# open-mmlab/Amphion

Hardware: AMD Instinct MI355X
Metric: audio samples/sec (HiFi-GAN V1 22.05 kHz generator, mel->wav) (higher is better)
Workload: dtype f32 (split-f16 MFMA: 3 x v_mfma_f32_32x32x16_f16 per term, f32 accumulate)

## Files before the change

amphion_amd/_lib.py:

```python
from __future__ import annotations

import ctypes
import os
import weakref
from ctypes import POINTER, c_char_p, c_float, c_int, c_int32, c_int64, c_size_t, c_void_p

_HERE = os.path.dirname(os.path.abspath(__file__))
LIB_PATH = os.environ.get("AMP_LIB_PATH") or os.path.join(_HERE, "lib", "libamphion_hip.so")

AMP_MAX_STAGES = 8
AMP_MAX_KERNELS = 8
AMP_MAX_DILATIONS = 8

AMP_ARCH_HIFIGAN, AMP_ARCH_BIGVGAN, AMP_ARCH_HIFIGAN_VITS = 0, 1, 2
AMP_ACT_LRELU, AMP_ACT_SNAKE, AMP_ACT_SNAKEBETA = 0, 1, 2
AMP_PRECISION_F32, AMP_PRECISION_F16X3 = 0, 1
AMP_CONV_OPT_PAD_REFLECT, AMP_CONV_OPT_TANH = 1, 2
AMP_PAD_REPLICATE, AMP_PAD_ZEROS, AMP_PAD_REFLECT = 0, 1, 2
AMP_PW_BIAS, AMP_PW_BIAS_GELU, AMP_PW_SCALE_RES = 0, 1, 2
PRECISIONS = {"f32": AMP_PRECISION_F32, "fp32": AMP_PRECISION_F32, "f16x3": AMP_PRECISION_F16X3}


class AmpError(RuntimeError):

# ... 219 lines not shown
    "amp_embed_tokens": (c_int, [c_void_p, c_void_p, c_void_p, c_int, c_int, c_int, c_int, c_float, c_void_p, c_void_p]),
    "amp_embed_sum_c": (c_int, [c_void_p, c_int, POINTER(c_void_p), POINTER(c_int), c_int, c_void_p, c_int, c_int, c_void_p, c_void_p, c_void_p]),
    "amp_embed_sum_check": (c_int, [c_void_p, c_void_p]),
    "amp_durations": (c_int, [c_void_p, c_void_p, c_int, c_int, c_float, c_void_p, c_void_p, c_void_p, c_void_p]),
    "amp_expand_path": (c_int, [c_void_p, c_void_p, c_void_p, c_void_p, c_int, c_int, c_int, c_int, c_void_p, c_void_p, c_void_p]),
    "amp_expand_path_strided": (c_int, [c_void_p, ctypes.c_longlong, c_void_p, c_void_p, c_void_p, c_int, c_int, c_int, c_int, c_void_p, c_void_p, c_void_p]),
    "amp_gauss_sample": (c_int, [c_void_p, c_void_p, c_void_p, c_size_t, c_float, c_void_p, c_void_p]),
    "amp_snake": (c_int, [c_void_p, c_int, c_int, c_int, c_void_p, c_void_p, c_int, c_void_p, c_void_p]),
    "amp_fir_upsample": (c_int, [c_void_p, c_int, c_int, c_int, c_void_p, c_int, c_int, c_void_p, c_void_p]),
    "amp_fir_filter": (c_int, [c_void_p, c_int, c_int, c_int, c_void_p, c_int, c_int, c_int, c_int, c_int, c_void_p, c_void_p]),
    "amp_wav_to_pcm16": (c_int, [c_void_p, c_int, c_int, ctypes.c_longlong, c_void_p, c_void_p, ctypes.c_longlong, c_void_p]),
    "amp_conv_set_option": (c_int, [c_void_p, c_int, c_int]),
    "amp_pair_forward": (c_int, [c_void_p, c_void_p, c_void_p, c_int, c_int, c_float, c_void_p, c_void_p]),
    "amp_resblock_forward": (c_int, [POINTER(c_void_p), POINTER(c_void_p), c_int, c_void_p, c_int, c_int, c_float, c_void_p, c_void_p]),
    "amp_set_resblock_fusion": (c_int, [c_int]),
    "amp_conv_destroy": (None, [c_void_p]),
    "amp_set_small_conv": (c_int, [c_int]),
    "amp_set_conv_blk": (c_int, [c_int]),
    "amp_set_conv_rg_fast": (c_int, [c_int]),
    "amp_set_pingpong": (c_int, [c_int]),
    "amp_set_conv_blk_narrow": (c_int, [c_int]),
    "amp_ampblock_forward": (c_int, [POINTER(c_void_p), POINTER(c_void_p), c_int, c_void_p, c_void_p, c_int, c_void_p, c_void_p,
                                     c_void_p, c_int, c_int, c_void_p, c_int, c_float, c_void_p]),
    "amp_set_ampblock_fusion": (c_int, [c_int]),
    "amp_conv_create_gated": (c_int, [c_int, c_int, c_int, c_int, c_void_p, c_void_p, POINTER(c_void_p)]),
    "amp_wn_forward": (c_int, [POINTER(c_void_p), POINTER(c_void_p), c_int, c_void_p, c_void_p, ctypes.c_longlong, c_void_p, c_int, c_int,
                               c_void_p, c_void_p, c_void_p]),
    "amp_wn_gate": (c_int, [c_void_p, c_void_p, ctypes.c_longlong, c_void_p, c_int, c_int, c_int, c_void_p]),
    "amp_wn_accumulate": (c_int, [c_void_p, c_void_p, c_void_p, c_void_p, c_int, c_int, c_int, c_int, c_int, c_void_p]),
    "amp_sequence_mask": (c_int, [c_void_p, c_void_p, c_int, c_int, c_int, c_void_p]),
# ... 136 lines not shown
```

amphion_amd/csrc/amp_host.h:

```cpp
#pragma once
#include <math.h>

#include <vector>

#include "amp_internal.h"

#define AMP_HIP(expr)                                                                  \
    do {                                                                               \
        hipError_t e__ = (expr);                                                       \
        if (e__ != hipSuccess) {                                                       \
            set_error("%s failed: %s (%s:%d)", #expr, hipGetErrorString(e__), __FILE__, __LINE__); \
            return AMP_ERR_HIP;                                                        \
        }                                                                              \
    } while (0)

#define AMP_RC(expr) do { int rc__ = (expr); if (rc__ != AMP_OK) return rc__; } while (0)

struct amp_conv {
    int transposed = 0, cin = 0, cout = 0, k = 0, stride = 1, dilation = 1, padding = 0;
    int M = 0, ntaps = 0, KT = 0, off0 = 0, dstep = 0, halo_left = 0, halo_right = 0, up = 1, up_pad = 0;
    int nchunks = 0;
    int precision = amp::PREC_F32;
    int pad_reflect = 0, tanh_out = 0;
    int out_pad = 0;
// ... 42 lines not shown
        return AMP_OK;
    }
    template <class T, class P>
    int upload(const std::vector<T>& v, P** out) { return upload(v.data(), v.size() * sizeof(T), (void**)out); }
};

int default_precision();

constexpr int kConvBlkDefault = 3;
constexpr int kConvRgFastDefault = 1;
constexpr int kPingPongDefault = 1;
struct Config {
    int pair_strips = -1;
    int strip_fit = -1;
    int rb_fusion = 1;
    int ampb_fusion = 1;
    int conv_blk = kConvBlkDefault;
    size_t group_bytes = 0;
    int small_conv = 1;
    int conv_rg_fast = 1;
    int pingpong = 1;
    int narrow_blk = 1;
    int rb_streams = -1;
    Config();
};
Config& cfg();

struct RangeGuard {
    unsigned* dev = nullptr;
    unsigned* host = nullptr;
// ... 53 lines not shown

int conv_build(amp_conv* c, const float* w, const float* bias);
int conv_run(const amp_conv* c, const float* x, int B, int T, float slope_in, const float* res, float slope_out, float* y, int mode, float div,
             hipStream_t stream, long long xbs = 0, const int* lens = nullptr, int len_mul = 1, ConvArgs* plan_small = nullptr,
             int* plan_ni = nullptr);
int next_rev(const int* lens);

bool pair_supported(const amp_conv* c1, const amp_conv* c2);
int pair_run(const amp_conv* c1, const amp_conv* c2, const float* x, int B, int T, float slope, float* y, int mode, float div,
             hipStream_t stream, const int* lens = nullptr, int len_mul = 1);
bool pair_strip_plan(int B, int T, int k, bool ragged, int* form, int* strip_len, int* spi, int* steps);
bool pair_tile_args(const amp_conv* c1, const amp_conv* c2, const float* x, int B, int T, float slope, float* y, int mode, float div,
                    const int* lens, int len_mul, PairArgs* out);

bool rb_supported(const amp_conv* const* c1, const amp_conv* const* c2, int np, int B, int T);
int rb_split(const amp_conv* const* c1, int np, int B, int T);
int rb_run(const amp_conv* const* c1, const amp_conv* const* c2, int np, const float* x, int B, int T, float slope, float* y, int mode,
           float div, hipStream_t stream, const int* lens = nullptr, int len_mul = 1, int first = 0, int count = -1);

struct ActParams {
    float* a_dev = nullptr;
    float* invb_dev = nullptr;
    float* fu_dev = nullptr;
    float* fd_dev = nullptr;
    float* fu2_dev = nullptr;
};
int act_params_upload(const float* alpha_dev, const float* beta_dev, int C, int logscale, const float* filt_up_host,
                      const float* filt_down_host, float** out);
bool ampb_supported(const amp_conv* const* c1, const amp_conv* const* c2, int np, const ActParams* acts, size_t nacts, int B, int T);
int ampb_run(const amp_conv* const* c1, const amp_conv* const* c2, int np, const ActParams* acts, const float* x, int B, int T, float* y,
             int mode, float div, hipStream_t stream, const int* lens = nullptr, int len_mul = 1);
// ... 3 lines not shown
```

amphion_amd/csrc/amp_internal.h:

```cpp
#pragma once
#include <hip/hip_runtime.h>
#include <stdarg.h>
#include <stdint.h>
#include <stdio.h>

#include <atomic>
#include <mutex>
#include <string>
#include <vector>

#include "amphion_hip.h"

namespace amp {

constexpr int KC = 8;
constexpr int KC16 = 16;

enum { PREC_F32 = 0, PREC_F16X3 = 1 };

struct ConvArgs {
    const float* x;
    const void* wp;
    const float* bias;
    const float* res;
// ... 65 lines not shown
};
hipError_t launch_pair3(const Pair3Args& p, hipStream_t stream);

constexpr int AMP_RB_MAX_PAIRS = 3;
struct RbArgs {
    const float* x;
    float* y;
    const void* wp1[AMP_RB_MAX_PAIRS];
    const float* bias1[AMP_RB_MAX_PAIRS];
    const void* wp2[AMP_RB_MAX_PAIRS];
    const float* bias2[AMP_RB_MAX_PAIRS];
    float sc1[AMP_RB_MAX_PAIRS], isc1[AMP_RB_MAX_PAIRS], sc2[AMP_RB_MAX_PAIRS], isc2[AMP_RB_MAX_PAIRS];
    int dil[AMP_RB_MAX_PAIRS];
    int np;
    int rh;
    int B, C, T;
    int tiles_per_item;
    int rev;
    float slope;
    int mode;
    float div;
    const int* lens;
    int len_mul;
    unsigned* range_flag;
};

constexpr int AMP_AMPB_MAX_STEPS = 6;
struct AmpbArgs {
    const float* x;
    float* y;
// ... 249 lines not shown
```

amphion_amd/csrc/conv_host.hip:

```cpp
#include <string.h>

#include <memory>
#include <type_traits>
#include <vector>

#include "amp_host.h"

namespace amp {

template <int... K> struct Taps { static constexpr int list[] = {K...}; };
using ConvTaps = Taps<1, 2, 3, 5, 7, 11>;
using BlkTaps = Taps<2, 3, 7, 11>;
using SmallTaps = Taps<1, 3, 5, 7, 11>;
using PairTaps = Taps<3, 5, 7, 11>;
using RbTaps = Taps<3, 5, 7, 11>;
using AmpbTaps = Taps<3, 5, 7, 11>;

template <int... K, typename R, typename F>
static R with_taps(Taps<K...>, int k, R dflt, F&& f) {
    R r = dflt;
    (void)((k == K && (r = f(std::integral_constant<int, K>{}), true)) || ...);
    return r;
}

// ... 380 lines not shown
    *out = a;
    return true;
}

static int rb_fusion_mode() { return cfg().rb_fusion; }
static int rb_form(int C, int k) {
    const int m = rb_fusion_mode();
    if (m == 0) return -1;
    if (m == 3) return (C == 32 || (C == 64 && k <= 5)) ? 0 : 1;
    if (m == 2) return 1;
    if (C == 32) return k >= 11 ? 1 : 0;
    if (C == 64) return k <= 5 ? 0 : 1;
    if (C == 128) return 1;
    return -1;
}
constexpr long long kRbMinWorkgroups = 256;

bool rb_supported(const amp_conv* const* c1, const amp_conv* const* c2, int np, int B, int T) {
    if (np < 1 || np > AMP_RB_MAX_PAIRS) return false;
    int max_dil = 1, rh = 0;
    for (int p = 0; p < np; ++p) {
        if (!c1[p] || !c2[p] || !pair_supported(c1[p], c2[p])) return false;
        if (c1[p]->cin != c1[0]->cin || c1[p]->k != c1[0]->k) return false;
        max_dil = c1[p]->dilation > max_dil ? c1[p]->dilation : max_dil;
        rh += (c1[p]->k - 1) / 2 * (c1[p]->dilation + 1);
    }
    const int form = rb_form(c1[0]->cin, c1[0]->k);
    if (form < 0) return false;
    const int W = rb_tile(c1[0]->k, c1[0]->cin, max_dil, form);
    if (W <= 0 || W - 2 * rh < W / 2) return false;
    const int NT = W - 2 * rh;
    if (rb_fusion_mode() == 1 && (long long)B * ((T + NT - 1) / NT) < kRbMinWorkgroups) return false;
    return true;
}

int rb_split(const amp_conv* const* c1, int np, int B, int T) {
    if (np != 3 || rb_fusion_mode() != 1) return 0;
    int max_dil = 1, rh = 0;
    for (int p = 0; p < np; ++p) {
        max_dil = c1[p]->dilation > max_dil ? c1[p]->dilation : max_dil;
        rh += (c1[p]->k - 1) / 2 * (c1[p]->dilation + 1);
    }
    const int W = rb_tile(c1[0]->k, c1[0]->cin, max_dil, rb_form(c1[0]->cin, c1[0]->k));
    const int NT = W - 2 * rh;
    if (W <= 0 || 5 * NT >= 4 * W) return 0;
    if ((long long)B * ((T + NT - 1) / NT) < 1024) return 0;
    return 2;
}

int rb_run(const amp_conv* const* c1, const amp_conv* const* c2, int np, const float* x, int B, int T, float slope, float* y, int mode,
           float div, hipStream_t stream, const int* lens, int len_mul, int first, int count) {
    if (x == y) { set_error("rb_run: x and y must not alias"); return AMP_ERR_INVALID; }
    if (slope > 1.f) { set_error("rb_run: leaky_relu slope %g > 1 is outside the fused kernels", (double)slope); return AMP_ERR_UNSUPPORTED; }
    RbArgs a{};
    a.x = x; a.y = y;
    a.np = count < 0 ? np - first : count;
    c1 += first;
    c2 += first;
    int max_dil = 1;
    for (int p = 0; p < a.np; ++p) {
        a.wp1[p] = c1[p]->wp_dev; a.bias1[p] = c1[p]->bias_dev; a.wp2[p] = c2[p]->wp_dev; a.bias2[p] = c2[p]->bias_dev;
        a.sc1[p] = 16.f * c1[p]->wscale; a.isc1[p] = 1.f / a.sc1[p];
        a.sc2[p] = 16.f * c2[p]->wscale; a.isc2[p] = 1.f / a.sc2[p];
        a.dil[p] = c1[p]->dilation;
        a.rh += (c1[p]->k - 1) / 2 * (c1[p]->dilation + 1);
        max_dil = c1[p]->dilation > max_dil ? c1[p]->dilation : max_dil;
    }
    for (int p = a.np; p < AMP_RB_MAX_PAIRS; ++p) {
        a.wp1[p] = a.wp1[0]; a.bias1[p] = a.bias1[0]; a.wp2[p] = a.wp2[0]; a.bias2[p] = a.bias2[0]; a.dil[p] = 1;
    }
    a.B = B; a.C = c1[0]->cin; a.T = T;
    const int form = rb_form(a.C, c1[0]->k);
    const int W = rb_tile(c1[0]->k, a.C, max_dil, form);
    const int NT = W - 2 * a.rh;
    a.tiles_per_item = (T + NT - 1) / NT;
    a.slope = slope; a.mode = mode; a.div = div;
    a.lens = lens; a.len_mul = len_mul;
    a.range_flag = range_flag_for_current_device();
    a.rev = next_rev(lens);
    AMP_HIP(launch_rb(c1[0]->k, a, form, stream));
    return AMP_OK;
}

static int ampb_fusion_mode() { return cfg().ampb_fusion; }
static int ampb_form(int C, int k) {
    const int m = ampb_fusion_mode();
    if (m == 0) return -1;
    if (m == 3) return C == 32 ? 0 : 1;
    if (m == 2) return 1;
    if (C == 32) return k >= 11 ? 1 : 0;
    if (C == 64) return k <= 3 ? 1 : -1;
    return -1;
}
constexpr long long kAmpbMinWorkgroups = 256;

// ... 220 lines not shown
}

int amp_resblock_forward(const amp_conv* const* c1, const amp_conv* const* c2, int n_pairs, const float* x_dev, int B, int T,
                         float slope, float* y_dev, void* stream) {
    if (!c1 || !c2 || !x_dev || !y_dev) { set_error("amp_resblock_forward: null argument"); return AMP_ERR_INVALID; }
    if (B <= 0 || T <= 0 || n_pairs < 1 || n_pairs > AMP_RB_MAX_PAIRS) { set_error("amp_resblock_forward: B=%d T=%d n_pairs=%d", B, T, n_pairs); return AMP_ERR_INVALID; }
    for (int p = 0; p < n_pairs; ++p) if (!c1[p] || !c2[p]) { set_error("amp_resblock_forward: null conv handle"); return AMP_ERR_INVALID; }
    if (!rb_supported(c1, c2, n_pairs, B, T)) {
        set_error("amp_resblock_forward: block (C=%d k=%d, %d pairs, B=%d T=%d) is not covered by the whole-resblock kernel under the "
                  "current amp_set_resblock_fusion mode", c1[0]->cin, c1[0]->k, n_pairs, B, T);
        return AMP_ERR_UNSUPPORTED;
    }
    return rb_run(c1, c2, n_pairs, x_dev, B, T, slope, y_dev, 0, 1.f, (hipStream_t)stream);
}

int amp_ampblock_forward(const amp_conv* const* c1, const amp_conv* const* c2, int n_pairs, const float* alpha_dev,
                         const float* beta_dev, int logscale, const float* filt_up_host, const float* filt_down_host,
                         const float* x_dev, int B, int T, float* y_dev, int mode, float div, void* stream) {
    if (!c1 || !c2 || !alpha_dev || !filt_up_host || !filt_down_host || !x_dev || !y_dev) { set_error("amp_ampblock_forward: null argument"); return AMP_ERR_INVALID; }
    if (B <= 0 || T <= 0 || n_pairs < 1 || 2 * n_pairs > AMP_AMPB_MAX_STEPS || mode < 0 || mode > 2) {
        set_error("amp_ampblock_forward: B=%d T=%d n_pairs=%d mode=%d", B, T, n_pairs, mode);
        return AMP_ERR_INVALID;
    }
    if (x_dev == y_dev) { set_error("amp_ampblock_forward: x and y must not alias (tiles read each other's halo)"); return AMP_ERR_INVALID; }
    for (int p = 0; p < n_pairs; ++p) if (!c1[p] || !c2[p]) { set_error("amp_ampblock_forward: null conv handle"); return AMP_ERR_INVALID; }
    const int C = c1[0]->cin, na = 2 * n_pairs;
    float* scratch[AMP_AMPB_MAX_STEPS] = {};
    ActParams acts[AMP_AMPB_MAX_STEPS];
    int rc = AMP_OK;
    for (int i = 0; i < na && rc == AMP_OK; ++i) {
// ... 42 lines not shown
```

amphion_amd/csrc/generator.hip:

```cpp
#include <math.h>
#include <stdio.h>

#include <map>
#include <memory>
#include <mutex>
#include <string>
#include <vector>

#include "amp_host.h"

using namespace amp;

struct HostTensor {
    std::vector<int64_t> shape;
    std::vector<float> data;
    size_t numel() const { size_t n = 1; for (auto s : shape) n *= (size_t)s; return n; }
};

struct ResBlock {
    int k = 0;
    std::vector<int> dil;
    std::vector<std::unique_ptr<amp_conv>> c1, c2;
    std::vector<ActParams> acts;
};
// ... 540 lines not shown
    *ran = true;
    return AMP_OK;
}

static int wait_before_last(hipEvent_t wait, hipStream_t sj) {
    if (wait) AMP_HIP(hipStreamWaitEvent(sj, wait, 0));
    return AMP_OK;
}

static int run_resblock1(const Stage& s, const ResBlock& rb, const RbBufs& b, int mode_last, hipEvent_t wait, hipStream_t sj) {
    const int B = s.B, t = s.t;
    const float nk = (float)s.g->d.n_kernels;
    const int nd = (int)rb.dil.size();
    RbPtrs q(rb);
    if (q.n && rb_supported(q.c1, q.c2, nd, B, t)) {
        const int sp = rb_split(q.c1, nd, B, t);
        if (sp > 0) AMP_RC(rb_run(q.c1, q.c2, nd, s.U, B, t, kLreluSlope, b.R, 0, 1.f, sj, s.lens, s.lm, 0, sp));
        AMP_RC(wait_before_last(wait, sj));
        return rb_run(q.c1, q.c2, nd, sp > 0 ? b.R : s.U, B, t, kLreluSlope, b.XS, mode_last, nk, sj, s.lens, s.lm, sp, -1);
    }
    const float* cur = s.U;
    for (int p = 0; p < nd; ++p) {
        const bool last = p == nd - 1;
        const amp_conv *c1 = rb.c1[p].get(), *c2 = rb.c2[p].get();
        if (pair_supported(c1, c2)) {
            float* dst = last ? b.XS : (cur == b.R ? b.TMP : b.R);
            if (last) AMP_RC(wait_before_last(wait, sj));
            AMP_RC(pair_run(c1, c2, cur, B, t, kLreluSlope, dst, last ? mode_last : 0, nk, sj, s.lens, s.lm));
            cur = dst;
            continue;
        }
        if (cur == b.TMP) {
            AMP_HIP(hipMemcpyAsync(b.R, b.TMP, (size_t)B * s.C * t * sizeof(float), hipMemcpyDeviceToDevice, sj));
            cur = b.R;
// ... 246 lines not shown
```

amphion_amd/csrc/rb_f16x3.hip:

```cpp
#include "f16x3_device.h"

#ifndef AMP_KT
#error "compile with -DAMP_KT=<taps>"
#endif

namespace amp {


template <int KT, int WM, int WN, int NI, int RING = 0, int RB_G = 32>
__global__ __launch_bounds__(64 * WM * WN, 2) void rb_f16x3_kernel(const RbArgs a) {
    static_assert(RING == 0 || RING < KT, "a ring shorter than one chunk");
    constexpr int NTHR = 64 * WM * WN;
    constexpr int W = 32 * NI * WN;
    constexpr int WL = W + 2 * RB_G;
    constexpr int H2 = (KT - 1) / 2;
    constexpr int NCH = 2 * WM;
    constexpr int CHS = 4 * WL;
    constexpr int C = 32 * WM;
    static_assert(NI % 2 == 0, "B fragments are read in halves");
    extern __shared__ __attribute__((aligned(16))) uint4 smem4[];

    const int tid = threadIdx.x;
    const int lane = tid & 63;
    const int wave = __builtin_amdgcn_readfirstlane(tid >> 6);
    const int wm = wave / WN, wn = wave % WN;
    const int hi = lane >> 5, l31 = lane & 31;
    const int nbx = gridDim.x;
    int bx = tile_order(blockIdx.x, nbx, a.lens != nullptr, a.rev);
    const int item = bx / a.tiles_per_item;
    const int tile = bx - item * a.tiles_per_item;
    const int T = a.T;
    const int RH = a.rh;
    const int NT = W - 2 * RH;
    const int O0 = tile * NT;
    int Tv = T;
    if (a.lens) { const int l = a.lens[item] * a.len_mul; Tv = l < Tv ? l : Tv; }
    if (O0 >= Tv) return;
    const int q0 = O0 - RH;

    for (int i = tid; i < NCH * 4 * 2 * RB_G; i += NTHR) {
        const int row = i / (2 * RB_G), g = i - row * (2 * RB_G);
        smem4[row * WL + (g < RB_G ? g : W + g)] = make_uint4(0u, 0u, 0u, 0u);
    }

    const int colw = wn * (32 * NI) + l31;
    int qcl[NI];
    bool qok[NI];
#pragma unroll
    for (int t = 0; t < NI; ++t) {
        const int q = q0 + colw + 32 * t;
        qok[t] = (q >= 0) && (q < Tv);
        qcl[t] = q < 0 ? 0 : (q < T ? q : T - 1);
    }
    const float* xr = a.x + (size_t)item * C * T + (size_t)(32 * wm + 16 * hi) * T;
    f32x16 rv[NI];
#pragma unroll
    for (int t = 0; t < NI; ++t)
// ... 2 lines not shown

    constexpr size_t MBS = (size_t)NCH * (KT * 128);
    constexpr int NA = RING > 0 ? RING : KT;
    Frag a_h[NA], a_l[NA];
    const int wlane = (lane & 32) | (16 * ((lane >> 2) & 1) + 4 * ((lane >> 3) & 3) + (lane & 3));
    {
        const uint4* w0 = static_cast<const uint4*>(a.wp1[0]) + (size_t)wm * MBS + wlane;
#pragma unroll
        for (int g = 0; g < NA; ++g) {
            a_h[g].u = w0[g * 128];
            a_l[g].u = w0[g * 128 + 64];
        }
    }
    AMP_PIN_VMEM();

    float range_max = 0.f;
    const float kpos = 16.f, kneg = 16.f * a.slope;
    auto stage_x = [&]() __attribute__((always_inline)) {
#pragma unroll
        for (int t = 0; t < NI; ++t) {
            const int col = RB_G + colw + 32 * t;
            const bool ok = qok[t];
            const int o4 = (2 * wm + hi) * CHS + col;
#pragma unroll
            for (int o = 0; o < 2; ++o) {
                struct { uint2 u; } fh0, fl0, fh1, fl1;
                stage4_f16(ok ? rv[t][8 * o + 0] : 0.f, ok ? rv[t][8 * o + 1] : 0.f, ok ? rv[t][8 * o + 2] : 0.f,
                           ok ? rv[t][8 * o + 3] : 0.f, kpos, kneg, range_max, fh0.u, fl0.u);
                stage4_f16(ok ? rv[t][8 * o + 4] : 0.f, ok ? rv[t][8 * o + 5] : 0.f, ok ? rv[t][8 * o + 6] : 0.f,
                           ok ? rv[t][8 * o + 7] : 0.f, kpos, kneg, range_max, fh1.u, fl1.u);
                smem4[o4 + o * WL] = make_uint4(fh0.u.x, fh0.u.y, fh1.u.x, fh1.u.y);
                smem4[o4 + o * WL + 2 * WL] = make_uint4(fl0.u.x, fl0.u.y, fl1.u.x, fl1.u.y);
// ... 41 lines not shown
                AMP_PIN_VMEM();
            }
        }
    };

    stage_x();
    __syncthreads();

    const int np = a.np;
#pragma unroll 1
    for (int p = 0; p < AMP_RB_MAX_PAIRS; ++p) {
        if (p < np) {
            const bool last = (p + 1 == np);
            conv(a.wp1[p], a.bias1[p], a.sc1[p], a.dil[p], a.wp2[p]);
            __syncthreads();
            {
                const float i1 = a.isc1[p];
                const float slope = a.slope;
#pragma unroll
                for (int t = 0; t < NI; ++t) {
                    const int o4 = (2 * wm + hi) * CHS + RB_G + colw + 32 * t;
#pragma unroll
                    for (int o = 0; o < 2; ++o) {
                        struct { uint2 u; } fh0, fl0, fh1, fl1;
                        seam4_f16(acc[t][8 * o + 0], acc[t][8 * o + 1], acc[t][8 * o + 2], acc[t][8 * o + 3], i1, slope, qok[t], range_max, fh0.u, fl0.u);
                        seam4_f16(acc[t][8 * o + 4], acc[t][8 * o + 5], acc[t][8 * o + 6], acc[t][8 * o + 7], i1, slope, qok[t], range_max, fh1.u, fl1.u);
                        smem4[o4 + o * WL] = make_uint4(fh0.u.x, fh0.u.y, fh1.u.x, fh1.u.y);
                        smem4[o4 + o * WL + 2 * WL] = make_uint4(fl0.u.x, fl0.u.y, fl1.u.x, fl1.u.y);
                    }
                }
// ... 41 lines not shown
                for (int r = 0; r < 16; ++r) yr[(size_t)r * T + qcl[t]] = rv[t][r];
            }
        }
    }
    if (a.range_flag && __any(range_max > 65504.f) && lane == 0) atomicOr(a.range_flag, 1u);
}

template <int KT, int WM, int WN, int NI, int RING = 0, int RB_G = 32>
static hipError_t launch_rb_one(const RbArgs& a, hipStream_t stream) {
    constexpr int W = 32 * NI * WN;
    const size_t lds = (size_t)2 * WM * 4 * (W + 2 * RB_G) * sizeof(uint4);
    if (hipError_t e = ensure_dynamic_lds<&rb_f16x3_kernel<KT, WM, WN, NI, RING, RB_G>>(lds); e != hipSuccess) return e;
    dim3 grid((unsigned)(a.B * a.tiles_per_item));
    note_kernel("rb_f16x3_kernel", KT, WM, WN, NI, RING, RB_G);
    note_work(grid.x, a.np * 2 * 2.0 * a.C * a.C * KT * (double)a.T * a.B / 1e9, 4.0 * a.B * (double)a.C * a.T * (2 + (a.mode ? 1 : 0)) / 1e6,
              "whole ResBlock C=%d k=%d T=%d B=%d: %d convs%s", a.C, KT, a.T, a.B, 2 * a.np, a.mode ? " +sum" : "");
    hipLaunchKernelGGL((rb_f16x3_kernel<KT, WM, WN, NI, RING, RB_G>), grid, dim3(64 * WM * WN), lds, stream, a);
    return hipGetLastError();
}

template <int KT>
int rb_tile(int C, int max_dil, int wide) {
    const int reach = (KT - 1) / 2 * max_dil;
    if (reach > 32) return 0;
    if (C == 32) return wide ? 1024 : 512;
    if (C == 64) return wide ? 512 : ((KT <= 5 && reach <= 16) ? 256 : 0);
    if (C == 128) return (wide && KT <= 5 && reach <= 16) ? 256 : 0;
    return 0;
}

template <int KT>
// ... 19 lines not shown
```

amphion_amd/csrc/runtime.hip:

```cpp
#include <stdarg.h>
#include <stdio.h>
#include <stdlib.h>
#include <string.h>

#include <mutex>
#include <string>

#include "amp_host.h"

namespace amp {

static thread_local char g_err[512] = "";

void set_error(const char* fmt, ...) {
    va_list ap;
    va_start(ap, fmt);
    vsnprintf(g_err, sizeof(g_err), fmt, ap);
    va_end(ap);
}

static RangeGuard g_guard[64];
__thread std::string* tl_kernel_log = nullptr;
__thread char tl_last_kernel[160] = "";
__thread int tl_conv_transposed = 0;
// ... 100 lines not shown
    if (g_precision < 0) {
        const char* e = getenv("AMP_PRECISION");
        g_precision = (e && (!strcmp(e, "f32") || !strcmp(e, "fp32"))) ? PREC_F32 : PREC_F16X3;
    }
    return g_precision;
}

Config::Config() {
    auto num = [](const char* name, int lo, int hi, int dflt) {
        const char* e = getenv(name);
        if (!e || !*e) return dflt;
        const int v = atoi(e);
        return (v < lo || v > hi) ? dflt : v;
    };
    rb_fusion = num("AMP_RB_FUSION", 0, 3, 1);
    ampb_fusion = num("AMP_AMPB_FUSION", 0, 3, 1);
    rb_streams = num("AMP_RB_STREAMS", -1, 1, -1);
    static const char* const kRemoved[][2] = {
        {"AMP_GROUP_MB", "amp_set_group_mb(megabytes)"}, {"AMP_PAIR_STRIP", "amp_set_pair_strips(mode)"}, {"AMP_CONV_BLK", "amp_set_conv_blk(mode)"},
        {"AMP_FUSE_PAIRS", "nothing (the fused pairs are the only form)"}, {"AMP_RB_SUM_FRAMES", "nothing"},
        {"AMP_RB_HORIZONTAL", "amp_set_resblock_streams(mode)"}, {"AMP_RB_HORIZONTAL_FRAMES", "amp_set_resblock_streams(mode)"}};
    for (const auto& r : kRemoved) {
        const char* e = getenv(r[0]);
        if (e && *e) fprintf(stderr, "libamphion_hip: the environment variable %s=%s is no longer read (removed in ABI 142); use %s\n", r[0], e, r[1]);
    }
}
Config& cfg() { static Config c; return c; }

int device_upload(const void* host, size_t bytes, void** out) {
    void* p = nullptr;
// ... 2 lines not shown
    if (e != hipSuccess) {
        (void)hipFree(p);
        set_error("hipMemcpy of %zu bytes to the device failed: %s", bytes, hipGetErrorString(e));
        return AMP_ERR_HIP;
    }
    *out = p;
    return AMP_OK;
}

}

using namespace amp;

extern "C" {

int amp_version(void) { return 159; }
const char* amp_last_error(void) { return g_err; }

int amp_set_precision(int precision) {
    if (precision != AMP_PRECISION_F32 && precision != AMP_PRECISION_F16X3) {
        set_error("amp_set_precision: unknown precision %d", precision);
        return AMP_ERR_INVALID;
    }
    g_precision = precision;
    return AMP_OK;
}

int amp_get_precision(void) { return default_precision(); }

int amp_device_count(void) {
    int n = 0;
// ... 52 lines not shown
    return AMP_OK;
}

int amp_set_conv_blk(int mode) {
    if (mode < -1 || mode > 3) { set_error("amp_set_conv_blk: mode %d (0 off, 1 | 2 chunks per staging round, 3 = 2 + k = 7 / 11, -1 default)", mode); return AMP_ERR_INVALID; }
    cfg().conv_blk = mode < 0 ? kConvBlkDefault : mode;
    return AMP_OK;
}

int amp_set_resblock_fusion(int mode) {
    if (mode < -1 || mode > 3) { set_error("amp_set_resblock_fusion: mode=%d", mode); return AMP_ERR_INVALID; }
    cfg().rb_fusion = mode < 0 ? 1 : mode;
    return AMP_OK;
}

int amp_set_ampblock_fusion(int mode) {
    if (mode < -1 || mode > 3) { set_error("amp_set_ampblock_fusion: mode=%d", mode); return AMP_ERR_INVALID; }
    cfg().ampb_fusion = mode < 0 ? 1 : mode;
    return AMP_OK;
}

int amp_range_check(void* stream_) {
    return range_check_sync(guard_for_current_device(), (hipStream_t)stream_, "amp_range_check");
}

}
```

include/amphion_hip.h:

```cpp
#ifndef AMPHION_HIP_H
#define AMPHION_HIP_H

#include <stddef.h>
#include <stdint.h>

#ifdef __cplusplus
extern "C" {
#endif

typedef enum amp_status {
    AMP_OK = 0,
    AMP_ERR_INVALID = -1,
    AMP_ERR_MISSING_WEIGHT = -2,
    AMP_ERR_HIP = -3,
    AMP_ERR_UNSUPPORTED = -4,
    AMP_ERR_STATE = -5,
    AMP_ERR_RANGE = -6
} amp_status;

typedef enum amp_arch {
    AMP_ARCH_HIFIGAN = 0,
    AMP_ARCH_BIGVGAN = 1,
    AMP_ARCH_HIFIGAN_VITS = 2
} amp_arch;
// ... 147 lines not shown
int amp_snake(const float* x_dev, int B, int C, int T, const float* alpha_dev, const float* beta_dev, int logscale,
              float* y_dev, void* stream);

int amp_wav_to_pcm16(const float* wav_dev, int B, int L, long long wav_stride, const int* lens_dev, int16_t* pcm_dev,
                     long long pcm_stride, void* stream);

typedef enum amp_conv_option { AMP_CONV_OPT_PAD_REFLECT = 1, AMP_CONV_OPT_TANH = 2 } amp_conv_option;
int amp_conv_set_option(amp_conv* c, int option, int value);

int amp_pair_forward(const amp_conv* c1, const amp_conv* c2, const float* x_dev, int B, int T, float slope,
                     float* y_dev, void* stream);

int amp_resblock_forward(const amp_conv* const* c1, const amp_conv* const* c2, int n_pairs, const float* x_dev, int B, int T,
                         float slope, float* y_dev, void* stream);
int amp_set_resblock_fusion(int mode);
int amp_set_resblock_streams(int mode);
int amp_gen_prepare_streams(amp_gen* g);

int amp_ampblock_forward(const amp_conv* const* c1, const amp_conv* const* c2, int n_pairs, const float* alpha_dev,
                         const float* beta_dev, int logscale, const float* filt_up_host, const float* filt_down_host,
                         const float* x_dev, int B, int T, float* y_dev, int mode, float div, void* stream);
int amp_set_ampblock_fusion(int mode);

void amp_conv_destroy(amp_conv* c);

int amp_set_small_conv(int on);

int amp_set_conv_blk(int mode);
int amp_set_conv_blk_narrow(int on);

// ... 291 lines not shown
```

Baseline: 150.4 million.

## Load first-conv halo into guard columns and cost-model resblock launch splits

The whole-resblock kernel can now fill its guard columns with real input data for the first conv instead of zeros. This shrinks the recomputed halo (rh) and widens the useful output per tile when the first dilation's reach fits in the guards. A cost model picks among 1, 2 or 3 launch splits of the three pairs, weighing workgroup waves against per-pair work and fixed trip overhead. In exchange it adds extra global loads for the guards, a guard re-zero after the first conv, a possible extra launch and temp buffer traffic, plus new API and env overrides.

```diff
diff --git a/amphion_amd/_lib.py b/amphion_amd/_lib.py
--- a/amphion_amd/_lib.py
+++ b/amphion_amd/_lib.py
@@ -257,6 +257,10 @@
     "amp_pair_forward": (c_int, [c_void_p, c_void_p, c_void_p, c_int, c_int, c_float, c_void_p, c_void_p]),
     "amp_resblock_forward": (c_int, [POINTER(c_void_p), POINTER(c_void_p), c_int, c_void_p, c_int, c_int, c_float, c_void_p, c_void_p]),
     "amp_set_resblock_fusion": (c_int, [c_int]),
+    "amp_set_rb_guards": (c_int, [c_int]),
+    "amp_set_rb_split_plan": (c_int, [c_int, POINTER(c_int)]),
+    "amp_rb_launch_plan": (c_int, [c_int, c_int, POINTER(c_int), c_int, c_int, c_int, c_int, POINTER(c_int), POINTER(c_int), POINTER(c_int), POINTER(c_int), POINTER(c_int)]),
+    "amp_resblock_forward_ex": (c_int, [POINTER(c_void_p), POINTER(c_void_p), c_int, c_void_p, c_int, c_int, c_float, c_void_p, c_int, c_float, c_void_p, c_void_p]),
     "amp_conv_destroy": (None, [c_void_p]),
     "amp_set_small_conv": (c_int, [c_int]),
     "amp_set_conv_blk": (c_int, [c_int]),
diff --git a/amphion_amd/csrc/amp_host.h b/amphion_amd/csrc/amp_host.h
--- a/amphion_amd/csrc/amp_host.h
+++ b/amphion_amd/csrc/amp_host.h
@@ -80,6 +80,8 @@
     int pair_strips = -1;
     int strip_fit = -1;
     int rb_fusion = 1;
+    int rb_guards = -1;
+    int rb_plan[3] = {0, 0, 0};
     int ampb_fusion = 1;
     int conv_blk = kConvBlkDefault;
     size_t group_bytes = 0;
@@ -163,7 +165,21 @@
                     const int* lens, int len_mul, PairArgs* out);
 
 bool rb_supported(const amp_conv* const* c1, const amp_conv* const* c2, int np, int B, int T);
-int rb_split(const amp_conv* const* c1, int np, int B, int T);
+struct RbGeom {
+    int W;
+    int rh0, rh;
+    int gx;
+    int NT0, NT;
+    int tiles0, tiles;
+};
+struct RbPlan {
+    int n;
+    int count[AMP_RB_MAX_PAIRS];
+};
+RbGeom rb_geometry(int C, int k, const int* dil, int first, int count, int T, int form);
+RbPlan rb_plan(int C, int k, const int* dil, int np, int B, int T, bool ragged);
+RbPlan rb_plan(const amp_conv* const* c1, int np, int B, int T, bool ragged);
+int rb_form_of(int C, int k);
 int rb_run(const amp_conv* const* c1, const amp_conv* const* c2, int np, const float* x, int B, int T, float slope, float* y, int mode,
            float div, hipStream_t stream, const int* lens = nullptr, int len_mul = 1, int first = 0, int count = -1);
 
diff --git a/amphion_amd/csrc/amp_internal.h b/amphion_amd/csrc/amp_internal.h
--- a/amphion_amd/csrc/amp_internal.h
+++ b/amphion_amd/csrc/amp_internal.h
@@ -103,6 +103,7 @@
     int dil[AMP_RB_MAX_PAIRS];
     int np;
     int rh;
+    int gx;
     int B, C, T;
     int tiles_per_item;
     int rev;
diff --git a/amphion_amd/csrc/conv_host.hip b/amphion_amd/csrc/conv_host.hip
--- a/amphion_amd/csrc/conv_host.hip
+++ b/amphion_amd/csrc/conv_host.hip
@@ -418,38 +418,95 @@
     if (C == 128) return 1;
     return -1;
 }
+int rb_form_of(int C, int k) { return rb_form(C, k); }
 constexpr long long kRbMinWorkgroups = 256;
+constexpr double kRbTripMacs = 235.0;
+
+static int rb_guard_columns(int C, int form) { return (C == 128 || (C == 64 && form == 0)) ? 16 : 32; }
+
+static bool rb_guards_wanted(int C, int k) {
+    const int m = cfg().rb_guards;
+    if (m >= 0) return m != 0;
+    return k >= 11 || (C == 64 && k >= 7);
+}
+
+RbGeom rb_geometry(int C, int k, const int* dil, int first, int count, int T, int form) {
+    RbGeom g{};
+    int max_dil = 1;
+    for (int p = first; p < first + count; ++p) {
+        max_dil = dil[p] > max_dil ? dil[p] : max_dil;
+        g.rh0 += (k - 1) / 2 * (dil[p] + 1);
+    }
+    g.W = form < 0 ? 0 : rb_tile(k, C, max_dil, form);
+    g.rh = g.rh0;
+    const int reach = (k - 1) / 2 * dil[first];
+    if (g.W > 0 && rb_guards_wanted(C, k) && reach <= rb_guard_columns(C, form)) { g.gx = 1; g.rh -= reach; }
+    g.NT = g.W - 2 * g.rh;
+    g.NT0 = g.W - 2 * g.rh0;
+    if (g.W > 0 && g.NT > 0) g.tiles = (T + g.NT - 1) / g.NT;
+    if (g.W > 0 && g.NT0 > 0) g.tiles0 = (T + g.NT0 - 1) / g.NT0;
+    return g;
+}
+static RbGeom rb_geometry(const amp_conv* const* c1, int first, int count, int T) {
+    int dil[AMP_RB_MAX_PAIRS] = {1, 1, 1};
+    for (int p = first; p < first + count && p < AMP_RB_MAX_PAIRS; ++p) dil[p] = c1[p]->dilation;
+    return rb_geometry(c1[0]->cin, c1[0]->k, dil, first, count, T, rb_form(c1[0]->cin, c1[0]->k));
+}
 
 bool rb_supported(const amp_conv* const* c1, const amp_conv* const* c2, int np, int B, int T) {
     if (np < 1 || np > AMP_RB_MAX_PAIRS) return false;
-    int max_dil = 1, rh = 0;
     for (int p = 0; p < np; ++p) {
         if (!c1[p] || !c2[p] || !pair_supported(c1[p], c2[p])) return false;
         if (c1[p]->cin != c1[0]->cin || c1[p]->k != c1[0]->k) return false;
-        max_dil = c1[p]->dilation > max_dil ? c1[p]->dilation : max_dil;
-        rh += (c1[p]->k - 1) / 2 * (c1[p]->dilation + 1);
-    }
-    const int form = rb_form(c1[0]->cin, c1[0]->k);
-    if (form < 0) return false;
-    const int W = rb_tile(c1[0]->k, c1[0]->cin, max_dil, form);
-    if (W <= 0 || W - 2 * rh < W / 2) return false;
-    const int NT = W - 2 * rh;
-    if (rb_fusion_mode() == 1 && (long long)B * ((T + NT - 1) / NT) < kRbMinWorkgroups) return false;
+    }
+    const RbGeom g = rb_geometry(c1, 0, np, T);
+    if (g.W <= 0 || g.NT0 < g.W / 2) return false;
+    if (rb_fusion_mode() == 1 && (long long)B * g.tiles0 < kRbMinWorkgroups) return false;
     return true;
 }
 
-int rb_split(const amp_conv* const* c1, int np, int B, int T) {
-    if (np != 3 || rb_fusion_mode() != 1) return 0;
-    int max_dil = 1, rh = 0;
-    for (int p = 0; p < np; ++p) {
-        max_dil = c1[p]->dilation > max_dil ? c1[p]->dilation : max_dil;
-        rh += (c1[p]->k - 1) / 2 * (c1[p]->dilation + 1);
-    }
-    const int W = rb_tile(c1[0]->k, c1[0]->cin, max_dil, rb_form(c1[0]->cin, c1[0]->k));
-    const int NT = W - 2 * rh;
-    if (W <= 0 || 5 * NT >= 4 * W) return 0;
-    if ((long long)B * ((T + NT - 1) / NT) < 1024) return 0;
-    return 2;
+RbPlan rb_plan(int C, int k, const int* dil, int np, int B, int T, bool ragged) {
+    RbPlan best{1, {np, 0, 0}};
+    if (np != 3) return best;
+    const int* f = cfg().rb_plan;
+    if (f[0] > 0) {
+        RbPlan forced{0, {0, 0, 0}};
+        for (int i = 0; i < 3 && f[i] > 0; ++i) forced.count[forced.n++] = f[i];
+        return forced;
+    }
+    if (rb_fusion_mode() != 1) return best;
+    const int form = rb_form(C, k);
+    const RbGeom whole = rb_geometry(C, k, dil, 0, np, T, form);
+    if (whole.W <= 0 || whole.NT0 <= 0) return best;
+    const long long wg0 = (long long)B * whole.tiles0;
+    if (wg0 < 1024) return best;
+    if (5 * whole.NT0 < 4 * whole.W) best = RbPlan{2, {2, 1, 0}};
+    if (ragged || !rb_guards_wanted(C, k)) return best;
+    const long long slots = 256 * (form == 0 ? 2 : 1);
+    const double trip = kRbTripMacs / ((double)C * k);
+    auto cost = [&](const RbPlan& pl) {
+        double c = 0.0;
+        for (int l = 0, first = 0; l < pl.n; first += pl.count[l++]) {
+            const RbGeom g = rb_geometry(C, k, dil, first, pl.count[l], T, form);
+            if (g.W <= 0 || g.NT <= 0) return -1.0;
+            c += (double)(((long long)B * g.tiles + slots - 1) / slots) * (2.0 * pl.count[l] + trip);
+        }
+        return c;
+    };
+    double best_cost = cost(best);
+    const RbPlan cands[] = {{1, {3, 0, 0}}, {2, {2, 1, 0}}, {2, {1, 2, 0}}, {3, {1, 1, 1}}};
+    const int min_launches = best.n;
+    for (const RbPlan& pl : cands) {
+        if (pl.n < min_launches || (pl.n == 3 && wg0 < 2048)) continue;
+        const double c = cost(pl);
+        if (c >= 0.0 && (best_cost < 0.0 || c < best_cost)) { best_cost = c; best = pl; }
+    }
+    return best;
+}
+RbPlan rb_plan(const amp_conv* const* c1, int np, int B, int T, bool ragged) {
+    int dil[AMP_RB_MAX_PAIRS] = {1, 1, 1};
+    for (int p = 0; p < np && p < AMP_RB_MAX_PAIRS; ++p) dil[p] = c1[p]->dilation;
+    return rb_plan(c1[0]->cin, c1[0]->k, dil, np, B, T, ragged);
 }
 
 int rb_run(const amp_conv* const* c1, const amp_conv* const* c2, int np, const float* x, int B, int T, float slope, float* y, int mode,
@@ -459,30 +516,27 @@
     RbArgs a{};
     a.x = x; a.y = y;
     a.np = count < 0 ? np - first : count;
+    const RbGeom g = rb_geometry(c1, first, a.np, T);
+    if (g.W <= 0 || g.NT <= 0) { set_error("rb_run: pairs [%d, %d) have no whole-resblock tile", first, first + a.np); return AMP_ERR_UNSUPPORTED; }
     c1 += first;
     c2 += first;
-    int max_dil = 1;
     for (int p = 0; p < a.np; ++p) {
         a.wp1[p] = c1[p]->wp_dev; a.bias1[p] = c1[p]->bias_dev; a.wp2[p] = c2[p]->wp_dev; a.bias2[p] = c2[p]->bias_dev;
         a.sc1[p] = 16.f * c1[p]->wscale; a.isc1[p] = 1.f / a.sc1[p];
         a.sc2[p] = 16.f * c2[p]->wscale; a.isc2[p] = 1.f / a.sc2[p];
         a.dil[p] = c1[p]->dilation;
-        a.rh += (c1[p]->k - 1) / 2 * (c1[p]->dilation + 1);
-        max_dil = c1[p]->dilation > max_dil ? c1[p]->dilation : max_dil;
     }
     for (int p = a.np; p < AMP_RB_MAX_PAIRS; ++p) {
         a.wp1[p] = a.wp1[0]; a.bias1[p] = a.bias1[0]; a.wp2[p] = a.wp2[0]; a.bias2[p] = a.bias2[0]; a.dil[p] = 1;
     }
     a.B = B; a.C = c1[0]->cin; a.T = T;
-    const int form = rb_form(a.C, c1[0]->k);
-    const int W = rb_tile(c1[0]->k, a.C, max_dil, form);
-    const int NT = W - 2 * a.rh;
-    a.tiles_per_item = (T + NT - 1) / NT;
+    a.rh = g.rh; a.gx = g.gx;
+    a.tiles_per_item = g.tiles;
     a.slope = slope; a.mode = mode; a.div = div;
     a.lens = lens; a.len_mul = len_mul;
     a.range_flag = range_flag_for_current_device();
     a.rev = next_rev(lens);
-    AMP_HIP(launch_rb(c1[0]->k, a, form, stream));
+    AMP_HIP(launch_rb(c1[0]->k, a, rb_form(a.C, c1[0]->k), stream));
     return AMP_OK;
 }
 
@@ -733,6 +787,32 @@
     return rb_run(c1, c2, n_pairs, x_dev, B, T, slope, y_dev, 0, 1.f, (hipStream_t)stream);
 }
 
+int amp_resblock_forward_ex(const amp_conv* const* c1, const amp_conv* const* c2, int n_pairs, const float* x_dev, int B, int T, float slope,
+                            float* y_dev, int mode, float div, float* tmp_dev, void* stream) {
+    if (!c1 || !c2 || !x_dev || !y_dev) { set_error("amp_resblock_forward_ex: null argument"); return AMP_ERR_INVALID; }
+    if (B <= 0 || T <= 0 || n_pairs < 1 || n_pairs > AMP_RB_MAX_PAIRS || mode < 0 || mode > 2) {
+        set_error("amp_resblock_forward_ex: B=%d T=%d n_pairs=%d mode=%d", B, T, n_pairs, mode);
+        return AMP_ERR_INVALID;
+    }
+    for (int p = 0; p < n_pairs; ++p) if (!c1[p] || !c2[p]) { set_error("amp_resblock_forward_ex: null conv handle"); return AMP_ERR_INVALID; }
+    if (!rb_supported(c1, c2, n_pairs, B, T)) {
+        set_error("amp_resblock_forward_ex: block (C=%d k=%d, %d pairs, B=%d T=%d) is not covered by the whole-resblock kernel under the "
+                  "current amp_set_resblock_fusion mode", c1[0]->cin, c1[0]->k, n_pairs, B, T);
+        return AMP_ERR_UNSUPPORTED;
+    }
+    const RbPlan pl = rb_plan(c1, n_pairs, B, T, false);
+    if (pl.n > 1 && !tmp_dev) { set_error("amp_resblock_forward_ex: a plan of %d launches needs tmp_dev", pl.n); return AMP_ERR_INVALID; }
+    const size_t be = (size_t)B * c1[0]->cin * T;
+    const float* cur = x_dev;
+    int first = 0;
+    for (int l = 0; l + 1 < pl.n; first += pl.count[l++]) {
+        float* dst = cur == tmp_dev ? tmp_dev + be : tmp_dev;
+        AMP_RC(rb_run(c1, c2, n_pairs, cur, B, T, slope, dst, 0, 1.f, (hipStream_t)stream, nullptr, 1, first, pl.count[l]));
+        cur = dst;
+    }
+    return rb_run(c1, c2, n_pairs, cur, B, T, slope, y_dev, mode, div, (hipStream_t)stream, nullptr, 1, first, -1);
+}
+
 int amp_ampblock_forward(const amp_conv* const* c1, const amp_conv* const* c2, int n_pairs, const float* alpha_dev,
                          const float* beta_dev, int logscale, const float* filt_up_host, const float* filt_down_host,
                          const float* x_dev, int B, int T, float* y_dev, int mode, float div, void* stream) {
diff --git a/amphion_amd/csrc/generator.hip b/amphion_amd/csrc/generator.hip
--- a/amphion_amd/csrc/generator.hip
+++ b/amphion_amd/csrc/generator.hip
@@ -578,10 +578,16 @@
     const int nd = (int)rb.dil.size();
     RbPtrs q(rb);
     if (q.n && rb_supported(q.c1, q.c2, nd, B, t)) {
-        const int sp = rb_split(q.c1, nd, B, t);
-        if (sp > 0) AMP_RC(rb_run(q.c1, q.c2, nd, s.U, B, t, kLreluSlope, b.R, 0, 1.f, sj, s.lens, s.lm, 0, sp));
+        const RbPlan pl = rb_plan(q.c1, nd, B, t, s.lens != nullptr);
+        const float* cur = s.U;
+        int first = 0;
+        for (int l = 0; l + 1 < pl.n; first += pl.count[l++]) {
+            float* dst = cur == b.R ? b.TMP : b.R;
+            AMP_RC(rb_run(q.c1, q.c2, nd, cur, B, t, kLreluSlope, dst, 0, 1.f, sj, s.lens, s.lm, first, pl.count[l]));
+            cur = dst;
+        }
         AMP_RC(wait_before_last(wait, sj));
-        return rb_run(q.c1, q.c2, nd, sp > 0 ? b.R : s.U, B, t, kLreluSlope, b.XS, mode_last, nk, sj, s.lens, s.lm, sp, -1);
+        return rb_run(q.c1, q.c2, nd, cur, B, t, kLreluSlope, b.XS, mode_last, nk, sj, s.lens, s.lm, first, -1);
     }
     const float* cur = s.U;
     for (int p = 0; p < nd; ++p) {
diff --git a/amphion_amd/csrc/rb_f16x3.hip b/amphion_amd/csrc/rb_f16x3.hip
--- a/amphion_amd/csrc/rb_f16x3.hip
+++ b/amphion_amd/csrc/rb_f16x3.hip
@@ -38,9 +38,43 @@
     if (O0 >= Tv) return;
     const int q0 = O0 - RH;
 
-    for (int i = tid; i < NCH * 4 * 2 * RB_G; i += NTHR) {
-        const int row = i / (2 * RB_G), g = i - row * (2 * RB_G);
-        smem4[row * WL + (g < RB_G ? g : W + g)] = make_uint4(0u, 0u, 0u, 0u);
+    float range_max = 0.f;
+    const float kpos = 16.f, kneg = 16.f * a.slope;
+    auto zero_guards = [&]() __attribute__((always_inline)) {
+        for (int i = tid; i < NCH * 4 * 2 * RB_G; i += NTHR) {
+            const int row = i / (2 * RB_G), g = i - row * (2 * RB_G);
+            smem4[row * WL + (g < RB_G ? g : W + g)] = make_uint4(0u, 0u, 0u, 0u);
+        }
+    };
+    constexpr int ZRS = NTHR / (8 * RB_G);
+    static_assert(NTHR % (8 * RB_G) == 0 && (NCH * 4) % ZRS == 0, "the guard words of a row tile the workgroup");
+    auto rezero_guards = [&]() __attribute__((always_inline)) {
+        const int r = tid & (8 * RB_G - 1), g = r >> 2;
+        unsigned* pz = reinterpret_cast<unsigned*>(smem4) + ((tid / (8 * RB_G)) * WL + (g < RB_G ? g : W + g)) * 4 + (r & 3);
+#pragma unroll
+        for (int it = 0; it < NCH * 4 / ZRS; ++it) pz[it * ZRS * WL * 4] = 0u;
+    };
+    if (a.gx) {
+        const float* xg = a.x + (size_t)item * C * T;
+#pragma unroll 1
+        for (int i = tid; i < NCH * 2 * 2 * RB_G; i += NTHR) {
+            const int co = i / (2 * RB_G), g = i - co * (2 * RB_G);
+            const int lc = g < RB_G ? g : W + g;
+            const int q = q0 - RB_G + lc;
+            const bool ok = (q >= 0) && (q < Tv);
+            const float* src = xg + (size_t)(8 * co) * T + (q < 0 ? 0 : (q < T ? q : T - 1));
+            float v[8];
+#pragma unroll
+            for (int e = 0; e < 8; ++e) v[e] = src[(size_t)e * T];
+            struct { uint2 u; } fh0, fl0, fh1, fl1;
+            stage4_f16(ok ? v[0] : 0.f, ok ? v[1] : 0.f, ok ? v[2] : 0.f, ok ? v[3] : 0.f, kpos, kneg, range_max, fh0.u, fl0.u);
+            stage4_f16(ok ? v[4] : 0.f, ok ? v[5] : 0.f, ok ? v[6] : 0.f, ok ? v[7] : 0.f, kpos, kneg, range_max, fh1.u, fl1.u);
+            const int o4 = (co >> 1) * CHS + (co & 1) * WL + lc;
+            smem4[o4] = make_uint4(fh0.u.x, fh0.u.y, fh1.u.x, fh1.u.y);
+            smem4[o4 + 2 * WL] = make_uint4(fl0.u.x, fl0.u.y, fl1.u.x, fl1.u.y);
+        }
+    } else {
+        zero_guards();
     }
 
     const int colw = wn * (32 * NI) + l31;
@@ -73,8 +107,6 @@
     }
     AMP_PIN_VMEM();
 
-    float range_max = 0.f;
-    const float kpos = 16.f, kneg = 16.f * a.slope;
     auto stage_x = [&]() __attribute__((always_inline)) {
 #pragma unroll
         for (int t = 0; t < NI; ++t) {
@@ -146,6 +178,7 @@
             const bool last = (p + 1 == np);
             conv(a.wp1[p], a.bias1[p], a.sc1[p], a.dil[p], a.wp2[p]);
             __syncthreads();
+            if (p == 0 && a.gx) rezero_guards();
             {
                 const float i1 = a.isc1[p];
                 const float slope = a.slope;
@@ -217,7 +250,7 @@
     dim3 grid((unsigned)(a.B * a.tiles_per_item));
     note_kernel("rb_f16x3_kernel", KT, WM, WN, NI, RING, RB_G);
     note_work(grid.x, a.np * 2 * 2.0 * a.C * a.C * KT * (double)a.T * a.B / 1e9, 4.0 * a.B * (double)a.C * a.T * (2 + (a.mode ? 1 : 0)) / 1e6,
-              "whole ResBlock C=%d k=%d T=%d B=%d: %d convs%s", a.C, KT, a.T, a.B, 2 * a.np, a.mode ? " +sum" : "");
+              "whole ResBlock C=%d k=%d T=%d B=%d%s rh=%d: %d convs%s", a.C, KT, a.T, a.B, a.gx ? " guards=x" : "", a.rh, 2 * a.np, a.mode ? " +sum" : "");
     hipLaunchKernelGGL((rb_f16x3_kernel<KT, WM, WN, NI, RING, RB_G>), grid, dim3(64 * WM * WN), lds, stream, a);
     return hipGetLastError();
 }
diff --git a/amphion_amd/csrc/runtime.hip b/amphion_amd/csrc/runtime.hip
--- a/amphion_amd/csrc/runtime.hip
+++ b/amphion_amd/csrc/runtime.hip
@@ -138,6 +138,15 @@
         return (v < lo || v > hi) ? dflt : v;
     };
     rb_fusion = num("AMP_RB_FUSION", 0, 3, 1);
+    rb_guards = num("AMP_RB_GUARDS", -1, 1, -1);
+    if (const char* e = getenv("AMP_RB_SPLIT_PLAN")) {
+        int v[3] = {0, 0, 0};
+        const int n = sscanf(e, "%d,%d,%d", &v[0], &v[1], &v[2]);
+        int sum = 0;
+        for (int i = 0; i < 3; ++i) sum += (i < n && v[i] > 0) ? v[i] : 0;
+        if (n >= 1 && sum == 3 && v[0] > 0 && (n < 2 || v[1] > 0) && (n < 3 || v[2] > 0))
+            for (int i = 0; i < 3; ++i) rb_plan[i] = i < n ? v[i] : 0;
+    }
     ampb_fusion = num("AMP_AMPB_FUSION", 0, 3, 1);
     rb_streams = num("AMP_RB_STREAMS", -1, 1, -1);
     static const char* const kRemoved[][2] = {
@@ -170,7 +179,7 @@
 
 extern "C" {
 
-int amp_version(void) { return 159; }
+int amp_version(void) { return 160; }
 const char* amp_last_error(void) { return g_err; }
 
 int amp_set_precision(int precision) {
@@ -253,6 +262,40 @@
     return AMP_OK;
 }
 
+int amp_set_rb_guards(int mode) {
+    if (mode < -1 || mode > 1) { set_error("amp_set_rb_guards: %d (-1 the policy, 0 never: zero guards, 1 wherever the first conv's reach fits)", mode); return AMP_ERR_INVALID; }
+    cfg().rb_guards = mode;
+    return AMP_OK;
+}
+
+int amp_set_rb_split_plan(int n, const int* counts) {
+    int v[3] = {0, 0, 0}, sum = 0;
+    if (n < 0 || n > 3 || (n > 0 && !counts)) { set_error("amp_set_rb_split_plan: n=%d (0 the plan, 1 .. 3 launches)", n); return AMP_ERR_INVALID; }
+    for (int i = 0; i < n; ++i) { v[i] = counts[i]; sum += v[i]; if (v[i] < 1) sum = -99; }
+    if (n > 0 && sum != 3) { set_error("amp_set_rb_split_plan: the launches must hold 1+ pairs each and 3 together"); return AMP_ERR_INVALID; }
+    for (int i = 0; i < 3; ++i) cfg().rb_plan[i] = v[i];
+    return AMP_OK;
+}
+
+int amp_rb_launch_plan(int C, int k, const int* dilations, int n_pairs, int B, int T, int ragged, int* n_launches, int* pairs, int* gx,
+                       int* out_columns, int* tiles_per_item) {
+    if (B < 1 || T < 1 || n_pairs < 1 || n_pairs > AMP_RB_MAX_PAIRS || !dilations || !n_launches || !pairs || !gx || !out_columns || !tiles_per_item) {
+        set_error("amp_rb_launch_plan: B=%d T=%d n_pairs=%d or a null pointer", B, T, n_pairs);
+        return AMP_ERR_INVALID;
+    }
+    const int form = rb_form_of(C, k);
+    int dil[AMP_RB_MAX_PAIRS] = {1, 1, 1};
+    for (int p = 0; p < n_pairs; ++p) dil[p] = dilations[p];
+    const RbPlan pl = rb_plan(C, k, dil, n_pairs, B, T, ragged != 0);
+    *n_launches = pl.n;
+    for (int l = 0, first = 0; l < pl.n; first += pl.count[l++]) {
+        const RbGeom g = rb_geometry(C, k, dil, first, pl.count[l], T, form);
+        if (g.W <= 0 || g.NT <= 0) { set_error("amp_rb_launch_plan: no whole-resblock kernel for C=%d k=%d under the current fusion mode", C, k); return AMP_ERR_UNSUPPORTED; }
+        pairs[l] = pl.count[l]; gx[l] = g.gx; out_columns[l] = g.NT; tiles_per_item[l] = g.tiles;
+    }
+    return AMP_OK;
+}
+
 int amp_set_ampblock_fusion(int mode) {
     if (mode < -1 || mode > 3) { set_error("amp_set_ampblock_fusion: mode=%d", mode); return AMP_ERR_INVALID; }
     cfg().ampb_fusion = mode < 0 ? 1 : mode;
diff --git a/include/amphion_hip.h b/include/amphion_hip.h
--- a/include/amphion_hip.h
+++ b/include/amphion_hip.h
@@ -185,6 +185,12 @@
 int amp_resblock_forward(const amp_conv* const* c1, const amp_conv* const* c2, int n_pairs, const float* x_dev, int B, int T,
                          float slope, float* y_dev, void* stream);
 int amp_set_resblock_fusion(int mode);
+int amp_set_rb_guards(int mode);
+int amp_set_rb_split_plan(int n, const int* counts);
+int amp_rb_launch_plan(int C, int k, const int* dilations, int n_pairs, int B, int T, int ragged, int* n_launches, int* pairs, int* gx,
+                       int* out_columns, int* tiles_per_item);
+int amp_resblock_forward_ex(const amp_conv* const* c1, const amp_conv* const* c2, int n_pairs, const float* x_dev, int B, int T, float slope,
+                            float* y_dev, int mode, float div, float* tmp_dev, void* stream);
 int amp_set_resblock_streams(int mode);
 int amp_gen_prepare_streams(amp_gen* g);
 
```

Result: faster. 152.1 million (median of 6 runs) (+1.1%).
